# slcs-jsc/jurassic-gpu

Measured on AMD Instinct MI355X. Metric: rays/s (radiance spectra/s) for limb EGA forward model, higher is better.
Workload: dtype f64; 1 GPU; limb_1e6; rays_total=1000000, channels=4, emitters=5, tables=synthetic 33p x 10T x ~203u per (gas, channel), fp32

## Files before the change

include/jurassic_hip.h:

```cpp
#ifndef JURASSIC_HIP_H
#define JURASSIC_HIP_H

#include "jurassic_abi.h"

#ifdef __cplusplus
extern "C" {
#endif

void formod(ctl_t const *ctl, atm_t *atm, obs_t *obs);
void formod_GPU(ctl_t const *ctl, atm_t *atm, obs_t *obs);
void formod_pencil(ctl_t const *ctl, atm_t *atm, obs_t *obs, int const ir);
void formod_contrib(ctl_t const *ctl, atm_t *atm, obs_t *obs, obs_t *contrib);
void formod_fov(ctl_t const *ctl, obs_t *obs);

void intpol_atm(ctl_t *ctl, atm_t *atm_dest, atm_t *atm_src);

typedef struct { size_t size1, size2, tda; double *data; void *block; int owner; } jur_gsl_matrix_t;
void kernel(ctl_t const *ctl, atm_t *atm, obs_t *obs, jur_gsl_matrix_t *k);

enum {
  JUR_OK = 0,
  JUR_EINVAL = -1,
  JUR_EIO = -2,
  JUR_ENOMEM = -3,
// ... 59 lines not shown
int  jur_curtis_godson_host(jur_model_t *m, long nr, double const *const geom[7],
                            double *cgp, double *cgt, double *cgu, double *const tp[3], int *np_out);

int  jur_fov_read_shape(char const *filename, int *n, double *dz, double *w);
int  jur_fov_apply(int nd, long nr, double const *time, double const *vpz, double *rad, double *tau, long ld,
                   int n, double const *dz, double const *w);

int  jur_fov_apply_device(jur_model_t *m, long nr, double const *d_time, double const *d_vpz, double *d_rad,
                          double *d_tau, int n, double const *dz, double const *w, void *stream);

int  jur_intpol_atm(ctl_t const *ctl, atm_t *dest, atm_t const *src, int device);

int  jur_model_reserve(jur_model_t *m, long nr);

long jur_model_workspace_bytes(jur_model_t const *m);
int  jur_model_chunk_rays(jur_model_t const *m);
long jur_model_table_bytes(jur_model_t const *m);
int  jur_device_info(int device, char *pci_bus_id, int len, size_t *free_bytes, size_t *total_bytes);
int  jur_model_set_chunk_rays(jur_model_t *m, int rays);
int  jur_model_set_sort_rays(jur_model_t *m, int on);
int  jur_model_set_trace_multiple(jur_model_t *m, int mult);
int  jur_model_set_compact_workspace(jur_model_t *m, int on);
long jur_model_last_launches(jur_model_t const *m);
int  jur_model_set_workspace_budget(jur_model_t *m, long bytes);

int  jur_model_set_pencil(jur_model_t *m, long max_rays, int rays_per_group);
void jur_tune_trace(int lanes_per_ray);
void jur_tune_combine(int channels_per_group, int sync_segments, long min_lanes);

enum { JUR_ARITH_FAST = 0, JUR_ARITH_EXACT = 1 };
int  jur_model_set_arithmetic(jur_model_t *m, int mode);
int  jur_model_arithmetic(jur_model_t const *m);

int  jur_dropin_finalize(void);

int  jur_model_enable_timing(jur_model_t *m, int on);
int  jur_model_last_kernel_ms(jur_model_t *m, double out_ms[3], long out_launches[3]);
int  jur_model_last_pencil_ms(jur_model_t *m, double *out_ms, long *out_launches);
int  jur_model_last_contrib_ms(jur_model_t *m, double *out_ms, long *out_launches);

int jur_kat_ega_eps(jur_model_t *m, int ig, int id, long n, double const *tau, double const *t, double const *u,
                    double const *p, int mode, int chain, double *out);
int jur_kat_continua(jur_model_t *m, int id, long n, double const *p, double const *t, double const *q,
                     double const *u_co2, double const *u_h2o, double *out);
int jur_kat_update(jur_model_t *m, int id, long n, int what, double const *a, double const *b, double const *c,
                   double *rad, double *tau, double *src);
// ... 8 lines not shown
```

jurassic-gpu_amd/csrc/jur_internal.h:

```cpp
#ifndef JUR_INTERNAL_H
#define JUR_INTERNAL_H

#include <stdint.h>
#include "jurassic_hip.h"

#ifdef __cplusplus
extern "C" {
#endif

typedef struct { int a, b; } jur_int2;
typedef struct { float u, eps; } jur_ue_t;
typedef struct { float u0, e0, u1, e1; double du_de, de_du; } __attribute__((aligned(32))) jur_rec_t;
typedef struct { double p; int nt; int c0; } jur_lvl_t;
typedef struct { double t; int nu; int e0; } jur_crv_t;

typedef struct {
  double nu;
  double co2_cw296, co2_cw260, co2_cw230;
  double h2o_sc;
  double h2o_ratio;
  double h2o_lnr_hi, h2o_lnr_lo;
  double h2o_ctwfrn;
  double n2_b, n2_beta;
  double o2_b, o2_beta;
// ... 26 lines not shown
  int atm_sorted;
  double const *atm_time, *atm_z, *atm_lon, *atm_lat, *atm_p, *atm_t;
  double const *atm_q;
  double const *atm_k;
  double const *atm_pslope;
} jur_view_t;

typedef struct {
  int n;
  int stride;
  int stride_eps;
  long first;
  int const *order;
  double const *geom[7];
  double *tp[3];
  double *rad, *tau;
  int *np_out;
  int *np;
  double *tsurf;
  double *los;
  double *eps;
  int const *eps_off;
  int *status;
} jur_chunk_t;

int jurk_prepare_atm(jur_view_t const *v, double *d_pslope, void *stream);
int jurk_launch_trace(jur_view_t const *v, jur_chunk_t const *c, void *stream);
int jurk_launch_ega(jur_view_t const *v, jur_chunk_t const *c, void *stream);
int jurk_launch_combine(jur_view_t const *v, jur_chunk_t const *c, void *stream);
int jurk_launch_contrib(jur_view_t const *v, jur_chunk_t const *c, long nr, double *rad_c, double *tau_c, void *stream);
int jurk_tile_max(int n, int const *d_np, int *d_tile_np, void *stream);
int jurk_launch_kquot(long nq, long n, double const *d_rad, double const *d_h, double *d_kq, void *stream);
void jurk_tune_combine(int group, int sync, long min_lanes);
void jurk_tune_trace(int lanes);
int jurk_launch_cg(jur_view_t const *v, jur_chunk_t const *c, double *cgp, double *cgt, double *cgu, void *stream);
int jurk_fill_records(jur_ue_t const *ue, jur_rec_t *rec, long long n, void *stream);
long jurk_sort_tmp_bytes(long nr);
int jurk_sort_rays(jur_view_t const *v, int by_profile, long nr, double const *d_geom, long ld, int *d_order, void *tmp,
                   long tmp_bytes, void *stream);

long jurk_pencil_lds_bytes(jur_view_t const *v, int RB);
int jurk_launch_pencil(jur_view_t const *v, jur_chunk_t const *c, int RB, void *stream);

int jurk_launch_fov(long nr, int nd, double const *time, double const *vpz, double const *rad0, double const *tau0, double *rad,
                    double *tau, long ld, int n, double const *dz, double const *w, int *status, void *stream);

int jurk_launch_intpol(int ip, int ng, int nw, int ns, int nd_, int nx, double cx, double cz, double const *src, double const *x1,
                       int const *idx, int const *nz, double const *dst, double const *x0, double *out, void *stream);

int jurk_kat_ega(jur_view_t const *v, int g, int d, long n, double const *tau, double const *t, double const *u, double const *p,
                 int mode, int chain, double *out, void *stream);
int jurk_kat_continua(jur_view_t const *v, int d, long n, double const *p, double const *t, double const *q, double const *u_co2,
                      double const *u_h2o, double *out, void *stream);
int jurk_kat_update(jur_view_t const *v, int d, long n, int what, double const *a, double const *b, double const *c, double *rad,
// ... 63 lines not shown
```

jurassic-gpu_amd/csrc/jur_kernels.hip:

```cpp

#include <hip/hip_runtime.h>
#include <hipcub/hipcub.hpp>
#include <cstdlib>
#include <mutex>
#include "jur_internal.h"

#define NLOS JUR_NLOS
#define TBLNS JUR_TBLNS

namespace {

__device__ __forceinline__ double c01(double x) { return (x > 1.) ? 1. : ((x < 0.) ? 0. : x); }
__device__ __forceinline__ double c01_num(double x) { return __builtin_fmax(__builtin_fmin(x, 1.), 0.); }

__device__ __forceinline__ double lip(double x0, double y0, double x1, double y1, double x) {
  return y0 + (x - x0) * (y1 - y0) / (x1 - x0);
}

__device__ __forceinline__ double div_rcp(double a, double b, double r) {
  double const q = a * r;
  return __builtin_fma(__builtin_fma(-b, q, a), r, q);
}
__device__ __forceinline__ double lip_rcp(double x0, double y0, double x1, double y1, double x, double r) {
  return y0 + div_rcp((x - x0) * (y1 - y0), x1 - x0, r);
// ... 1007 lines not shown
  int const npair = v.nd * v.ng;
  BlockItem const bi = xcd_block_item((int)blockIdx.x, nrb, npair);
  int const rb = bi.rb, pr = bi.item;
  if (rb < 0) return;
  int const d = pr / v.ng, g = pr - d * v.ng;
  int const r = rb * blockDim.x + threadIdx.x;
  int const pair_idx = g * v.nd + d;
  jur_int2 const pd = v.pair[pair_idx];
  if (pd.a < 2) return;
  PairDesc<LDS> D{v.lvl, v.crv, v.ue + v.pair_e0[pair_idx], (unsigned)pd.b, 0u, 0u, 0u};
  if constexpr (RCPB) D.recb = v.rec + v.pair_e0[pair_idx];
  stage_pair<LDS, RCPB>(v, pd, D);
  if (r >= c.n) return;
  int const nfield = JUR_F_K + v.nw + v.ng;
  int const tile = __builtin_amdgcn_readfirstlane(r >> 6);
  unsigned const lane = (unsigned)(r & 63);
  size_t const R = (size_t)nfield * 64;
  double const *const los_tile = c.los + (size_t)tile * los_tile_doubles(nfield);
  double const *const los_p = los_tile + JUR_F_P * 64, *const los_t = los_tile + JUR_F_T * 64,
               *const los_u = los_tile + (size_t)(JUR_F_K + v.nw + g) * 64;
  size_t const Re = (size_t)npair * 64;
  double *const out = c.eps + eps_tile_point0(c, tile) * Re + (size_t)pr * 64;
  int const np = c.np[r];
  double tau_path = 1.0;
  unsigned br = 0, ia = 0, ib = 0;
  constexpr bool AHEAD = RCPB || !WARM;
  double p_next = 0., t_next = 0.;
  if (AHEAD && np > 0) { p_next = ldg<double>(los_p, lane); t_next = ldg<double>(los_t, lane); }

  for (int ip = 0; ip < np; ++ip) {
    size_t const o = (size_t)ip * R;
    double p, t;
    if constexpr (AHEAD) {
      p = p_next; t = t_next;
      if (ip + 1 < np) { p_next = ldg<double>(los_p + o + R, lane); t_next = ldg<double>(los_t + o + R, lane); }
    } else { p = ldg<double>(los_p + o, lane); t = ldg<double>(los_t + o, lane); }
    double const u = ldg<double>(los_u + o, lane);
    if constexpr (RCPB) tau_path = ega_eps_warm<LDS, true, true>(v, pd, D, tau_path, t, u, p, br, ia, ib);
    else if constexpr (WARM) tau_path *= ega_eps_warm<LDS, false>(v, pd, D, tau_path, t, u, p, br, ia, ib);
    else tau_path *= ega_eps_exact<LDS>(v, pd, D, tau_path, t, u, p);
    st_stream(out + (size_t)ip * Re, lane, tau_path);
  }
}

struct SegmentIn { double p, t, ds, k, u_co2, q_h2o, u_h2o, pcur; };
__device__ __forceinline__ SegmentIn load_segment(double const *__restrict__ row, double const *__restrict__ trow, unsigned lane,
                                                  int f_k, int f_co2, int f_h2o, int ng, unsigned has_table) {
  SegmentIn in;
  in.p = ldg<double>(row + JUR_F_P * 64, lane);
  in.t = ldg<double>(row + JUR_F_T * 64, lane);
  in.ds = ldg<double>(row + JUR_F_DS * 64, lane);
  in.k = ldg<double>(row + (size_t)f_k * 64, lane);
  in.u_co2 = ldg<double>(row + (size_t)f_co2 * 64, lane);
  in.q_h2o = ldg<double>(row + JUR_F_QH2O * 64, lane);
  in.u_h2o = ldg<double>(row + (size_t)f_h2o * 64, lane);
  double tg[8];
#pragma unroll
  for (int k = 0; k < 8; k++) tg[k] = (k < ng && ((has_table >> k) & 1u)) ? ld_stream(trow + (size_t)k * 64, lane) : 1.0;
  double pcur = 1.0;
#pragma unroll
  for (int k = 0; k < 8; k++) pcur *= tg[k];
  for (int g0 = 8; g0 < ng; g0 += 8) {
#pragma unroll
    for (int k = 0; k < 8; k++) tg[k] = (g0 + k < ng && g0 + k < 32 && ((has_table >> (g0 + k)) & 1u)) ? ld_stream(trow + (size_t)(g0 + k) * 64, lane) : 1.0;
// ... 13 lines not shown
  double *const sr = reinterpret_cast<double *>(jur_lds);
  Exp2Lds const e2t{sr + TBLNS};
  {
    double const *const gsr = v.sr + (size_t)d * TBLNS;
    for (int i = threadIdx.x; i < TBLNS; i += blockDim.x) sr[i] = gsr[i];
    if (threadIdx.x < 64) sr[TBLNS + threadIdx.x] = JUR_EXP2_64[threadIdx.x];
    __syncthreads();
  }
  if (r >= c.n) return;
  long const ray = c.order ? (long)c.order[r] : c.first + r;
  int const nfield = JUR_F_K + v.nw + ng;
  int const tile = __builtin_amdgcn_readfirstlane(r >> 6);
  unsigned const lane = (unsigned)(r & 63);
  size_t const R = (size_t)nfield * 64, Re = (size_t)nd * ng * 64;
  double const *const los = c.los + (size_t)tile * los_tile_doubles(nfield);
  double const *const epsb = c.eps + eps_tile_point0(c, tile) * Re + (size_t)d * ng * 64;
  jur_chan_t const ch = v.chan[d];
  int const f_k = JUR_F_K + ch.window, f_u = JUR_F_K + v.nw;
  bool const do_co2 = (v.fourbit & 8) && ch.co2_on, do_h2o = (v.fourbit & 4) && ch.h2o_on,
             do_n2 = (v.fourbit & 2) && ch.n2_on, do_o2 = (v.fourbit & 1) && ch.o2_on;
  size_t const oidx = (size_t)ray * nd + d;
  bool const masked = !isfinite(c.rad[oidx]);
  double rad = 0.0, tau = 1.0, pprev = 1.0;
  int const np = c.np[r];
  unsigned has_table = 0;
  for (int g = 0; g < ng && g < 32; g++) has_table |= (v.pair[g * nd + d].a >= 2 ? 1u : 0u) << g;
  int const f_co2 = do_co2 ? f_u + v.ig_co2 : JUR_F_P, f_h2o = do_h2o ? f_u + v.ig_h2o : JUR_F_P;
  for (int ip = 0; ip < np; ++ip) {
    SegmentIn const in = load_segment(los + (size_t)ip * R, epsb + (size_t)ip * Re, lane, f_k, f_co2, f_h2o, ng, has_table);
    double beta_ds = in.k * in.ds;
    if (do_co2) beta_ds += ctm_co2(ch, in.p, in.t, in.u_co2);
    double const rt = rcp_t(in.t);
    if (do_h2o) beta_ds += ctm_h2o(e2t, ch, in.p, in.t, rt, in.q_h2o, in.u_h2o);
    if (do_n2) beta_ds += ctm_n2(e2t, ch, in.p, in.t, rt) * in.ds;
    if (do_o2) beta_ds += ctm_o2(e2t, ch, in.p, in.t, rt) * in.ds;
    double const tau_gas = segment_tau_gas(in.pcur, pprev);
    pprev = in.pcur;
    new_obs_step(e2t, tau_gas, beta_ds, planck_src(sr, in.t), rad, tau);
  }
  ray_epilogue(sr, ch.nu, c.tsurf[r], v.write_bbt, rad, tau);
  if (masked) rad = __builtin_nan("");
  c.rad[oidx] = rad;
  c.tau[oidx] = tau;
}

#ifndef JUR_COMBINE_WAVES
#define JUR_COMBINE_WAVES 8
// ... 2 lines not shown
  int const nd = v.nd, ng = v.ng;
  int const ncg = (nd + CG - 1) / CG, SUB = (int)(blockDim.x >> 6) / CG;
  BlockItem const bi = xcd_block_item((int)blockIdx.x, nsb, ncg);
  int const sb = bi.rb, cg = bi.item;
  if (sb < 0) return;
  int const w = __builtin_amdgcn_readfirstlane((int)(threadIdx.x >> 6)), lane = (int)(threadIdx.x & 63);
  int const cw = w % CG, sub = w / CG;
  int const d = cg * CG + cw;
  bool const live_wave = d < nd;
  double *const sr = reinterpret_cast<double *>(jur_lds) + (size_t)cw * TBLNS;
  int *const npmax_sh = reinterpret_cast<int *>(reinterpret_cast<double *>(jur_lds) + (size_t)CG * TBLNS);
  Exp2Lds const e2t{reinterpret_cast<double *>(jur_lds) + (size_t)CG * TBLNS + 2};
  if (threadIdx.x == 0) *npmax_sh = 0;
  if (threadIdx.x < 64) reinterpret_cast<double *>(jur_lds)[(size_t)CG * TBLNS + 2 + threadIdx.x] = JUR_EXP2_64[threadIdx.x];
  for (int k = 0; k < CG; k++) {
    if (cg * CG + k >= nd) break;
    double const *const gsr = v.sr + (size_t)(cg * CG + k) * TBLNS;
    double *const dst = reinterpret_cast<double *>(jur_lds) + (size_t)k * TBLNS;
    for (int i = threadIdx.x; i < TBLNS; i += blockDim.x) dst[i] = gsr[i];
  }
  __syncthreads();
  int const r = (sb * SUB + sub) * 64 + lane;
  bool const live = live_wave && r < c.n;
  int const np = live ? c.np[r] : 0;
  atomicMax(npmax_sh, np);
  __syncthreads();
  int const npmax = *npmax_sh;
  long const ray = live ? (c.order ? (long)c.order[r] : c.first + r) : 0;
  int const nfield = JUR_F_K + v.nw + ng;
  int const tile = sb * SUB + sub;
  size_t const R = (size_t)nfield * 64, Re = (size_t)nd * ng * 64;
  double const *const los = c.los + (size_t)tile * los_tile_doubles(nfield);
  int const dd = live_wave ? d : 0;
  double const *const epsb = c.eps + eps_tile_point0(c, tile) * Re + (size_t)dd * ng * 64;
  jur_chan_t const ch = v.chan[dd];
  int const f_k = JUR_F_K + ch.window, f_u = JUR_F_K + v.nw;
  bool const do_co2 = (v.fourbit & 8) && ch.co2_on, do_h2o = (v.fourbit & 4) && ch.h2o_on,
             do_n2 = (v.fourbit & 2) && ch.n2_on, do_o2 = (v.fourbit & 1) && ch.o2_on;
  size_t const oidx = (size_t)ray * nd + dd;
  bool const masked = live && !isfinite(c.rad[oidx]);
  double rad = 0.0, tau = 1.0, pprev = 1.0;
  unsigned has_table = 0;
  for (int g = 0; g < ng && g < 32; g++) has_table |= (v.pair[g * nd + dd].a >= 2 ? 1u : 0u) << g;
  int const f_co2 = do_co2 ? f_u + v.ig_co2 : JUR_F_P, f_h2o = do_h2o ? f_u + v.ig_h2o : JUR_F_P;
  for (int ip = 0; ip < npmax; ++ip) {
    if (ip < np) {
      SegmentIn const in = load_segment(los + (size_t)ip * R, epsb + (size_t)ip * Re, (unsigned)lane, f_k, f_co2, f_h2o, ng, has_table);
// ... 390 lines not shown
  }
}

__global__ __launch_bounds__(256) void jur_records_kernel(long long n, jur_ue_t const *__restrict__ ue, jur_rec_t *__restrict__ rec) {
  for (long long i = (long long)blockIdx.x * blockDim.x + threadIdx.x; i < n; i += (long long)gridDim.x * blockDim.x) {
    double const du = (double)ue[i + 1].u - (double)ue[i].u, de = (double)ue[i + 1].eps - (double)ue[i].eps;
    rec[i] = jur_rec_t{ue[i].u, ue[i].eps, ue[i + 1].u, ue[i + 1].eps, du / de, de / du};
  }
}

__global__ __launch_bounds__(256) void jur_kquot_kernel(long nq, long n, long nrnd, double const *__restrict__ rad,
                                                        double const *__restrict__ h, double *__restrict__ kq) {
  long const t = (long)blockIdx.x * blockDim.x + threadIdx.x;
  if (t >= nq * n) return;
  long const q = t / n, e = t - q * n;
  kq[t] = (rad[(e + 1) * nrnd + q] - rad[q]) / h[e];
}

__global__ __launch_bounds__(256) void jur_tilemax_kernel(int n, int const *__restrict__ np, int *__restrict__ tile_np) {
  int const r = blockIdx.x * blockDim.x + threadIdx.x;
  int m = r < n ? np[r] : 0;
  for (int o = 32; o > 0; o >>= 1) m = max(m, __shfl_xor(m, o));
  if ((threadIdx.x & 63) == 0 && (r >> 6) < (n + 63) / 64) tile_np[r >> 6] = m;
}

__global__ __launch_bounds__(256) void jur_raykey_kernel(long nr, long ld, double const *__restrict__ geom,
                                                         double const *__restrict__ atm_time, int atm_np, int by_profile,
                                                         unsigned long long *__restrict__ key, int *__restrict__ id) {
  long const r = (long)blockIdx.x * blockDim.x + threadIdx.x;
  if (r >= nr) return;
  double xo[3], xv[3], e[3];
  geo2cart(geom[1 * ld + r], geom[2 * ld + r], geom[3 * ld + r], xo);
  geo2cart(geom[4 * ld + r], geom[5 * ld + r], geom[6 * ld + r], xv);
  for (int i = 0; i < 3; i++) e[i] = xv[i] - xo[i];
  double const n = norm3(e);
  double h = norm3(xo) - JUR_RE;
  if (n > 0) {
    double s = 0;
    for (int i = 0; i < 3; i++) s -= xo[i] * e[i] / n;
    if (s > 0) h = sqrt(fmax(xo[0] * xo[0] + xo[1] * xo[1] + xo[2] * xo[2] - s * s, 0.)) - JUR_RE;
  }
  unsigned const fb = __float_as_uint((float)h);
  unsigned const ord = fb ^ ((fb >> 31) ? 0xffffffffu : 0x80000000u);
  unsigned long long slice = 0;
  if (by_profile) {
    double const time = geom[r];
// ... 282 lines not shown
  if (c->n <= 0) return 0;
  int const block = 256;
  int const nrb = (c->n + block - 1) / block;
  long const nitem = (long)v->nd * (v->ng + 1);
  if (((long)(nrb >> 3) + 1) * 8 * nitem * block >= (1L << 32)) return (int)hipErrorInvalidValue;
  unsigned const grid = xcd_grid(nrb, (int)nitem);
  hipLaunchKernelGGL(jur_contrib_kernel, dim3(grid), dim3(block), sizeof(double) * (JUR_TBLNS + 64), (hipStream_t)stream, *v, *c,
                     nrb, nr, rad_c, tau_c);
  return (int)hipGetLastError();
}

extern "C" int jurk_launch_kquot(long nq, long n, double const *d_rad, double const *d_h, double *d_kq, void *stream) {
  if (nq <= 0 || n <= 0) return 0;
  hipLaunchKernelGGL(jur_kquot_kernel, dim3((unsigned)((nq * n + 255) / 256)), dim3(256), 0, (hipStream_t)stream, nq, n, nq, d_rad, d_h, d_kq);
  return (int)hipGetLastError();
}

extern "C" int jurk_tile_max(int n, int const *d_np, int *d_tile_np, void *stream) {
  if (n <= 0) return 0;
  hipLaunchKernelGGL(jur_tilemax_kernel, dim3((unsigned)((n + 255) / 256)), dim3(256), 0, (hipStream_t)stream, n, d_np, d_tile_np);
  return (int)hipGetLastError();
}

extern "C" int jurk_launch_cg(jur_view_t const *v, jur_chunk_t const *c, double *cgp, double *cgt, double *cgu,
                              void *stream) {
  if (c->n <= 0 || v->ng <= 0) return 0;
  int const block = 256;
  long const pencils = (long)c->n * v->ng;
  unsigned const grid = (unsigned)((pencils * 64 + block - 1) / block);
  hipLaunchKernelGGL(jur_cg_kernel, dim3(grid), dim3(block), 0, (hipStream_t)stream, *v, *c, cgp, cgt, cgu);
  return (int)hipGetLastError();
}

static size_t align_up(size_t x) { return (x + 255) & ~(size_t)255; }

extern "C" long jurk_sort_tmp_bytes(long nr) {
  size_t cub = 0;
  if (hipcub::DeviceRadixSort::SortPairs(nullptr, cub, (unsigned long long const *)nullptr, (unsigned long long *)nullptr,
                                         (int const *)nullptr, (int *)nullptr, (int)nr) != hipSuccess)
    cub = 64 * (size_t)nr + (1 << 20);
  return (long)(2 * align_up(8 * (size_t)nr) + align_up(4 * (size_t)nr) + align_up(cub) + 256);
}

extern "C" int jurk_sort_rays(jur_view_t const *v, int by_profile, long nr, double const *d_geom, long ld, int *d_order, void *tmp,
                              long tmp_bytes, void *stream) {
  hipStream_t s = (hipStream_t)stream;
// ... 125 lines not shown
```

jurassic-gpu_amd/csrc/jur_model.c:

```c
#define _GNU_SOURCE
#include <math.h>
#include <stdio.h>
#include <stdlib.h>
#include <string.h>
#include <strings.h>
#include <pthread.h>
#include <unistd.h>
#include <sched.h>
#include <hip/hip_runtime_api.h>
#include "jur_internal.h"

#define HIPCHK(call)                                                                       \
  do {                                                                                     \
    hipError_t e_ = (call);                                                                \
    if (e_ != hipSuccess) {                                                                \
      jur_set_error("HIP error %d (%s) at %s:%d", (int)e_, hipGetErrorString(e_), __FILE__, __LINE__); \
      return JUR_EHIP;                                                                     \
    }                                                                                      \
  } while (0)

struct jur_model {
  int device;
  int shared_tables;
  ctl_t *ctl;
  jur_view_t view;
  long table_bytes;
  void *d_chan, *d_sr, *d_pair, *d_pair_e0, *d_lvl, *d_crv, *d_ue, *d_rec;
  int arith;
  void *d_atm;
  int atm_cap;
  int atm_slices;
  double atm_zmin, atm_zmax;
  int chunk_rays;
  int nfield;
  double *d_los;
  double *d_eps;
  long ws_budget;
  long ws_rays;
  long ws_trace_rays;
  int trace_mult;
  long use_rays, use_trace_rays;
  int *d_np;
  double *d_tsurf;
  int compact_ws;
  int use_compact;
  int *d_tile_np, *d_eps_off;
  int *h_tile;
  long n_launch_ega;
  int *d_status;
  long los_bytes;
  int sort_rays;
  int *d_order;
  void *d_sort_tmp;
  long order_cap, sort_tmp_bytes;
  double *d_io;
  int *d_io_np;
  long io_cap;
  int *h_status;
  double *h_io;
  long h_io_cap;
  double *h_pkg;
  double *h_atm;
  long h_atm_n, h_atm_cap;
  double h_atm_hydz;
  hipStream_t stream;
  hipStream_t stream2;
  hipEvent_t ev_mask, ev_trace;
  int host_call;
  hipEvent_t ev_done;
// ... 122 lines not shown
    }
    v->rec = (jur_rec_t const *)m->d_rec;
  }
  v->sorted_tables = fl.sorted;
  v->strict_tables = fl.strict;
  v->max_pair_curves = fl.max_pair_curves;
  m->table_bytes = (long)((sizeof(jur_ue_t) + (m->d_rec ? sizeof(jur_rec_t) : 0)) * fl.nentry + 16 * fl.ncurve + 16 * fl.nlevel + 8 * npair);
  jur_flat_free(&fl);
  if (rc) { jur_model_destroy(m); return rc; }
  v->chan = (jur_chan_t const *)m->d_chan;
  v->sr = (double const *)m->d_sr;
  v->pair = (jur_int2 const *)m->d_pair;
  v->pair_e0 = (long long const *)m->d_pair_e0;
  v->lvl = (jur_lvl_t const *)m->d_lvl;
  v->crv = (jur_crv_t const *)m->d_crv;
  v->ue = (jur_ue_t const *)m->d_ue;
  if ((rc = jur_model_set_arithmetic(m, getenv("JUR_EGA_NO_RCP") ? JUR_ARITH_EXACT : JUR_ARITH_FAST))) { jur_model_destroy(m); return rc; }

  m->nfield = JUR_F_K + v->nw + v->ng;
  m->chunk_rays = 1 << 21;
  m->sort_rays = 1;
  m->ws_budget = 128L << 30;
  m->compact_ws = getenv("JUR_NO_COMPACT_WS") ? 0 : 1;
  m->trace_mult = 1;
  m->pencil_rays = 10000;
  m->pencil_rb = 0;
  if (getenv("JUR_PENCIL_RAYS")) m->pencil_rays = atol(getenv("JUR_PENCIL_RAYS"));
  if (getenv("JUR_PENCIL_RB")) m->pencil_rb = atoi(getenv("JUR_PENCIL_RB"));
  if (getenv("JUR_CHUNK_RAYS") && atoi(getenv("JUR_CHUNK_RAYS")) >= 64) m->chunk_rays = (atoi(getenv("JUR_CHUNK_RAYS")) + 63) / 64 * 64;
  if (getenv("JUR_TRACE_MULT") && atoi(getenv("JUR_TRACE_MULT")) >= 1) m->trace_mult = atoi(getenv("JUR_TRACE_MULT"));
  if (getenv("JUR_WS_GIB") && atoi(getenv("JUR_WS_GIB")) >= 1) m->ws_budget = (long)atoi(getenv("JUR_WS_GIB")) << 30;
  if ((rc = create_streams(m))) { jur_model_destroy(m); return rc; }
  if ((rc = upload((void **)&m->d_status, NULL, sizeof(int)))) { jur_model_destroy(m); return rc; }
  if (hipMemset(m->d_status, 0, sizeof(int)) != hipSuccess) { jur_set_error("cannot clear the status word"); jur_model_destroy(m); return JUR_EHIP; }
  *out = m;
  return JUR_OK;
}

int jur_model_set_arithmetic(jur_model_t *m, int mode) {
  if (mode != JUR_ARITH_FAST && mode != JUR_ARITH_EXACT) { jur_set_error("set_arithmetic: JUR_ARITH_FAST or JUR_ARITH_EXACT"); return JUR_EINVAL; }
  jur_view_t *v = &m->view;
  int const lds_ok = v->max_pair_curves > 0 && 24L * JUR_TBLNP + 24L * v->max_pair_curves <= 48 * 1024;
  m->arith = mode;
  v->fast_arith = (mode == JUR_ARITH_FAST) && v->strict_tables && v->rec && lds_ok;
  return JUR_OK;
}
// ... 201 lines not shown
    return JUR_OK;
  }
  if ((long)(nrow * n) > m->h_atm_cap) {
    free(m->h_atm);
    m->h_atm = (double *)malloc(sizeof(double) * nrow * n);
    m->h_atm_cap = m->h_atm ? (long)(nrow * n) : 0;
  }
  m->h_atm_n = 0;
  if (m->h_atm) { memcpy(m->h_atm, h, sizeof(double) * nrow * n); m->h_atm_n = n; m->h_atm_hydz = m->ctl->hydz; }
  hydrostatic_rows(m, h, (size_t)n, 0, n);
  int const rc = upload_atm_rows(m, h, n);
  if (rc) m->h_atm_n = 0;
  free(h);
  return rc;
}

static void free_workspace(jur_model_t *m) {
  if (m->d_los) (void)hipFree(m->d_los);
  if (m->d_eps) (void)hipFree(m->d_eps);
  if (m->d_np) (void)hipFree(m->d_np);
  if (m->d_tsurf) (void)hipFree(m->d_tsurf);
  if (m->d_tile_np) (void)hipFree(m->d_tile_np);
  if (m->d_eps_off) (void)hipFree(m->d_eps_off);
  if (m->h_tile) (void)hipHostFree(m->h_tile);
  m->d_los = NULL; m->d_eps = NULL; m->d_np = NULL; m->d_tsurf = NULL; m->d_tile_np = NULL; m->d_eps_off = NULL; m->h_tile = NULL;
  m->los_bytes = 0; m->ws_rays = 0; m->ws_trace_rays = 0;
}

static int ensure_workspace(jur_model_t *m, long nr) {
  long const per_ray_los = (long)sizeof(double) * m->nfield * JUR_NLOS;
  long const per_ray_eps = (long)sizeof(double) * m->view.nd * (m->view.ng > 0 ? m->view.ng : 1) * JUR_NLOS;
  long budget = m->ws_budget;
  int asked = 0;
  for (int attempt = 0;; attempt++) {
    long R = m->chunk_rays;
    long const fit = budget / (per_ray_los + per_ray_eps);
    if (R > fit) R = fit / 64 * 64;
    if (R < 64) R = 64;
    if (nr <= R) R = (nr + 63) / 64 * 64;
    else {
      long const nchunk = (nr + R - 1) / R;
      R = ((nr + nchunk - 1) / nchunk + 63) / 64 * 64;
    }
    long mult = m->trace_mult > 0 ? m->trace_mult : 1;
    while (mult > 1 && (per_ray_los * mult + per_ray_eps) * R > budget) mult--;
    long Rt = R * mult;
    if (nr < Rt) Rt = (nr + R - 1) / R * R;
    int compact = 0;
    if (nr > R && m->compact_ws) {
      long Rt_c = (nr + 63) / 64 * 64;
      if (per_ray_los * Rt_c > budget / 2) Rt_c = budget / 2 / per_ray_los / 64 * 64;
      long R_c = (budget - per_ray_los * Rt_c) / per_ray_eps / 64 * 64;
      if (R_c > m->chunk_rays) R_c = m->chunk_rays;
      if (R_c >= 64 && Rt_c >= R_c) { R = R_c; Rt = Rt_c; compact = 1; }
    }
    if (R <= m->ws_rays && Rt <= m->ws_trace_rays) {
      m->use_rays = R;
      m->use_trace_rays = Rt;
      m->use_compact = compact;
      return JUR_OK;
    }
    if (!asked) {
      size_t free_b = 0, total_b = 0;
      asked = 1;
      if (hipMemGetInfo(&free_b, &total_b) == hipSuccess) {
        long const avail = (long)free_b + m->los_bytes - (2L << 30);
        if (avail > (64L << 20) && avail < budget) { budget = avail; continue; }
      } else (void)hipGetLastError();
    }
    free_workspace(m);
    hipError_t e = hipMalloc((void **)&m->d_los, (size_t)per_ray_los * Rt);
    if (e == hipSuccess) e = hipMalloc((void **)&m->d_eps, (size_t)per_ray_eps * R);
    if (e == hipSuccess) e = hipMalloc((void **)&m->d_np, sizeof(int) * Rt);
    if (e == hipSuccess) e = hipMalloc((void **)&m->d_tsurf, sizeof(double) * Rt);
    if (e == hipSuccess) e = hipMalloc((void **)&m->d_tile_np, sizeof(int) * (Rt / 64 + 1));
    if (e == hipSuccess) e = hipMalloc((void **)&m->d_eps_off, sizeof(int) * (Rt / 64 + 1));
    if (e == hipSuccess) e = hipHostMalloc((void **)&m->h_tile, sizeof(int) * 2 * (Rt / 64 + 1), hipHostMallocDefault);
    if (e == hipSuccess) {
      m->los_bytes = per_ray_los * Rt + per_ray_eps * R;
      m->ws_rays = R;
      m->ws_trace_rays = Rt;
      m->use_rays = R;
      m->use_trace_rays = Rt;
      m->use_compact = compact;
      return JUR_OK;
    }
    (void)hipGetLastError();
    free_workspace(m);
    if (R <= 64 || attempt >= 24) {
      jur_set_error("cannot allocate the workspace (%ld B per ray, even for %ld rays): %s", per_ray_los + per_ray_eps, R,
                    hipGetErrorString(e));
      return JUR_EHIP;
    }
    budget = (per_ray_los + per_ray_eps) * R / 2;
// ... 4 lines not shown
long jur_model_table_bytes(jur_model_t const *m) { return m->table_bytes; }

int jur_device_info(int device, char *pci_bus_id, int len, size_t *free_bytes, size_t *total_bytes) {
  int ndev = 0;
  if (hipGetDeviceCount(&ndev) != hipSuccess || device < 0 || device >= ndev) { jur_set_error("device %d not available", device); return JUR_ENODEV; }
  HIPCHK(hipSetDevice(device));
  if (pci_bus_id && len > 0) HIPCHK(hipDeviceGetPCIBusId(pci_bus_id, len, device));
  size_t f = 0, t = 0;
  HIPCHK(hipMemGetInfo(&f, &t));
  if (free_bytes) *free_bytes = f;
  if (total_bytes) *total_bytes = t;
  return JUR_OK;
}
int jur_model_device(jur_model_t const *m) { return m->device; }
int jur_model_nd(jur_model_t const *m) { return m->view.nd; }
void *jur_model_stream(jur_model_t const *m) { return (void *)m->stream; }
int *jur_model_status_word(jur_model_t const *m) { return m->d_status; }
void jur_model_cost_params(jur_model_t const *m, double *rayds, double *raydz, double *zmin, double *zmax) {
  *rayds = m->view.rayds; *raydz = m->view.raydz; *zmin = m->atm_zmin; *zmax = m->atm_zmax;
}
int jur_model_chunk_rays(jur_model_t const *m) { return m->chunk_rays; }
long jur_model_last_launches(jur_model_t const *m) { return m->n_launch_ega; }
int jur_model_set_compact_workspace(jur_model_t *m, int on) { m->compact_ws = on ? 1 : 0; return JUR_OK; }

int jur_model_set_sort_rays(jur_model_t *m, int on) { m->sort_rays = on ? 1 : 0; return JUR_OK; }

int jur_model_set_workspace_budget(jur_model_t *m, long bytes) {
  if (bytes < (64L << 20)) { jur_set_error("workspace budget below 64 MiB"); return JUR_EINVAL; }
  m->ws_budget = bytes;
  return JUR_OK;
}

int jur_model_set_trace_multiple(jur_model_t *m, int mult) {
  if (mult < 1 || mult > 64) { jur_set_error("trace multiple must be in 1..64"); return JUR_EINVAL; }
  m->trace_mult = mult;
  return JUR_OK;
}

int jur_model_set_chunk_rays(jur_model_t *m, int rays) {
  if (rays < 64 || rays > (1 << 22)) { jur_set_error("chunk_rays must be in 64..4194304"); return JUR_EINVAL; }
  m->chunk_rays = (rays + 63) / 64 * 64;
  return JUR_OK;
}

int jur_model_set_pencil(jur_model_t *m, long max_rays, int rays_per_group) {
  if (max_rays < 0 || rays_per_group < 0 || rays_per_group > 64) { jur_set_error("set_pencil: max_rays >= 0, rays_per_group in 0..64"); return JUR_EINVAL; }
// ... 156 lines not shown
  }
  rc = ensure_workspace(m, nr);
  if (rc) return rc;
  long const R = m->use_rays;
  int const *order = NULL;
  if (m->sort_rays && nr > 64) {
    rc = ensure_sort_buffers(m, nr);
    if (rc) return rc;
    int const by_profile = m->atm_slices > 1 && nr >= 1024L * m->atm_slices;
    int const e = jurk_sort_rays(&m->view, by_profile, nr, d_geom, ldg, m->d_order, m->d_sort_tmp, m->sort_tmp_bytes, s);
    if (e) { jur_set_error("ray sort failed: %s", hipGetErrorString((hipError_t)e)); return JUR_EHIP; }
    order = m->d_order;
  }
  long const Rt = m->use_trace_rays;
  m->n_launch_ega = 0;
#define TIMED(kind, launch, what)                                                              \
  do {                                                                                         \
    int const ti_ = (m->timing && m->ntimed < JUR_MAX_TIMED) ? m->ntimed++ : -1;               \
    if (ti_ >= 0) { m->evkind[ti_] = (kind); HIPCHK(hipEventRecord(m->evpool[2 * ti_], s)); } \
    int const e_ = (launch);                                                                   \
    if (e_) { jur_set_error(what " kernel launch failed: %s", hipGetErrorString((hipError_t)e_)); return JUR_EHIP; } \
    if (ti_ >= 0) HIPCHK(hipEventRecord(m->evpool[2 * ti_ + 1], s));                          \
  } while (0)
  for (long t0 = 0; t0 < nr; t0 += Rt) {
    jur_chunk_t c;
    long const nt = (nr - t0 < Rt) ? nr - t0 : Rt;
    c.stride = (int)Rt;
    c.stride_eps = (int)R;
    for (int k = 0; k < 7; k++) c.geom[k] = d_geom + (size_t)k * ldg;
    for (int k = 0; k < 3; k++) c.tp[k] = d_tp + (size_t)k * ldtp;
    c.rad = d_rad;
    c.tau = d_tau;
    c.np_out = d_np;
    c.eps = m->d_eps;
    c.status = d_status ? d_status : m->d_status;
    c.n = (int)nt;
    c.first = t0;
    c.order = order ? order + t0 : NULL;
    c.np = m->d_np;
    c.tsurf = m->d_tsurf;
    c.los = m->d_los;
    TIMED(0, jurk_launch_trace(&m->view, &c, s), "trace");
    if (m->host_call) {
      if (t0 == 0) HIPCHK(hipStreamWaitEvent(s, m->ev_mask, 0));
      if (t0 + Rt >= nr) HIPCHK(hipEventRecord(m->ev_trace, s));
    }
    c.eps_off = NULL;
    int compact = m->use_compact && nt > R;
    if (compact) {
      hipStreamCaptureStatus st = hipStreamCaptureStatusNone;
      if (hipStreamIsCapturing(s, &st) != hipSuccess) { (void)hipGetLastError(); st = hipStreamCaptureStatusNone; }
      if (st != hipStreamCaptureStatusNone) compact = 0;
    }
    if (compact) {
      long const ntile = (nt + 63) / 64, cap = R / 64 * JUR_NLOS;
      int *const h_np = m->h_tile, *const h_off = m->h_tile + (m->ws_trace_rays / 64 + 1);
      int const ek = jurk_tile_max((int)nt, m->d_np, m->d_tile_np, s);
      if (ek) { jur_set_error("tile kernel launch failed: %s", hipGetErrorString((hipError_t)ek)); return JUR_EHIP; }
// ... 3 lines not shown
      for (long t = 0; t < ntile; t++) total += h_np[t];
      long const nchunk = (total + cap - 1) / cap > 0 ? (total + cap - 1) / cap : 1;
      long const target = (total + nchunk - 1) / nchunk;
      for (long t = 0; t < ntile;) {
        long acc = 0, e = t;
        while (e < ntile && (e == t || (acc + h_np[e] <= cap && acc < target))) acc += h_np[e++];
        if (e < ntile && e - t >= 64) e = t + (e - t) / 32 * 32;
        acc = 0;
        for (long q = t; q < e; q++) { h_off[q] = (int)acc; acc += h_np[q]; h_np[q] = (q == t); }
        t = e;
      }
      HIPCHK(hipMemcpyAsync(m->d_eps_off, h_off, sizeof(int) * ntile, hipMemcpyHostToDevice, s));
      for (long t0c = 0; t0c < ntile;) {
        long t1c = t0c + 1;
        while (t1c < ntile && !h_np[t1c]) t1c++;
        long const s0 = t0c * 64, s1 = (t1c * 64 < nt) ? t1c * 64 : nt;
        c.n = (int)(s1 - s0);
        c.first = t0 + s0;
        c.order = order ? order + t0 + s0 : NULL;
        c.np = m->d_np + s0;
        c.tsurf = m->d_tsurf + s0;
        c.los = m->d_los + (size_t)s0 * JUR_NLOS * m->nfield;
        c.eps_off = m->d_eps_off + t0c;
        TIMED(1, jurk_launch_ega(&m->view, &c, s), "ega");
        if (co) TIMED(4, jurk_launch_contrib(&m->view, &c, nr, co->rad, co->tau, s), "contribution");
        TIMED(2, jurk_launch_combine(&m->view, &c, s), "combine");
        m->n_launch_ega++;
        t0c = t1c;
      }
      continue;
    }
    for (long s0 = 0; s0 < nt; s0 += R) {
      c.n = (int)((nt - s0 < R) ? nt - s0 : R);
      c.first = t0 + s0;
      c.order = order ? order + t0 + s0 : NULL;
      c.np = m->d_np + s0;
      c.tsurf = m->d_tsurf + s0;
      c.los = m->d_los + (size_t)s0 * JUR_NLOS * m->nfield;
      TIMED(1, jurk_launch_ega(&m->view, &c, s), "ega");
      if (co) TIMED(4, jurk_launch_contrib(&m->view, &c, nr, co->rad, co->tau, s), "contribution");
      TIMED(2, jurk_launch_combine(&m->view, &c, s), "combine");
      m->n_launch_ega++;
    }
  }
#undef TIMED
  return record_done(m, s);
}

void *jur_host_alloc(size_t bytes) {
  void *p = NULL;
  if (hipHostMalloc(&p, bytes ? bytes : 8, hipHostMallocDefault) != hipSuccess) {
    (void)hipGetLastError();
    jur_set_error("hipHostMalloc of %zu bytes failed", bytes);
    return NULL;
  }
  return p;
}
void jur_host_free(void *p) { if (p) (void)hipHostFree(p); }

static int is_pinned(void const *p) {
  hipPointerAttribute_t a;
  if (!p) return 0;
  if (hipPointerGetAttributes(&a, p) != hipSuccess) { (void)hipGetLastError(); return 0; }
  return a.type == hipMemoryTypeHost;
}

typedef struct { char *dst; char const *src; size_t n; } cpjob_t;
static void *cp_worker(void *a) { cpjob_t const *j = (cpjob_t const *)a; memcpy(j->dst, j->src, j->n); return NULL; }
// ... 882 lines not shown
```

jurassic-gpu_amd/jurassic_hip/lib.py:

```python
import ctypes as C
import os
import numpy as np
from . import abi

PKG = os.path.dirname(os.path.dirname(os.path.abspath(__file__)))
SO = os.environ.get("JURASSIC_HIP_SO",
                    os.path.join(PKG, "libjurassic_hip%s.so" % os.environ.get("JUR_SUFFIX", "")))
_lib = None
dp = C.POINTER(C.c_double)


class JurassicError(RuntimeError):
    pass


def lib():
    global _lib
    if _lib is None:
        if not os.path.exists(SO):
            raise JurassicError(f"{SO} not built: run `make -C jurassic-gpu_amd/csrc` "
                                "or __graft_entry__.build(); no CPU fallback exists")
        L = C.CDLL(SO)
        L.jur_last_error.restype = C.c_char_p
        L.jur_fov_read_shape.argtypes = [C.c_char_p, C.POINTER(C.c_int), dp, dp]
# ... 22 lines not shown
        L.jur_curtis_godson_host.argtypes = [C.c_void_p, C.c_long, C.POINTER(dp), dp, dp, dp, C.POINTER(dp), C.POINTER(C.c_int)]
        L.jur_fov_apply_device.argtypes = [C.c_void_p, C.c_long] + [C.c_void_p] * 4 + [C.c_int, dp, dp, C.c_void_p]
        L.jur_intpol_atm.argtypes = [C.c_void_p, C.c_void_p, C.c_void_p, C.c_int]
        L.intpol_atm.argtypes = [C.c_void_p] * 3
        L.intpol_atm.restype = None
        L.jur_host_alloc.restype = C.c_void_p
        L.jur_host_alloc.argtypes = [C.c_size_t]
        L.jur_host_free.argtypes = [C.c_void_p]
        L.jur_formod_device.argtypes = [C.c_void_p, C.c_long] + [C.c_void_p] * 7
        L.jur_formod_contrib_host.argtypes = [C.c_void_p, C.c_long, C.POINTER(dp), dp, dp, C.POINTER(dp), C.POINTER(C.c_int), dp, dp]
        L.jur_formod_contrib_device.argtypes = [C.c_void_p, C.c_long] + [C.c_void_p] * 9
        L.formod_contrib.argtypes = [C.c_void_p] * 4
        L.formod_contrib.restype = None
        L.jur_model_reserve.argtypes = [C.c_void_p, C.c_long]
        L.jur_model_workspace_bytes.restype = C.c_long
        L.jur_model_workspace_bytes.argtypes = [C.c_void_p]
        L.jur_model_table_bytes.restype = C.c_long
        L.jur_model_table_bytes.argtypes = [C.c_void_p]
        L.jur_device_info.argtypes = [C.c_int, C.c_char_p, C.c_int, C.POINTER(C.c_size_t), C.POINTER(C.c_size_t)]
        L.jur_model_chunk_rays.argtypes = [C.c_void_p]
        L.jur_model_last_launches.restype = C.c_long
        L.jur_model_last_launches.argtypes = [C.c_void_p]
        L.jur_model_set_compact_workspace.argtypes = [C.c_void_p, C.c_int]
        L.jur_model_set_chunk_rays.argtypes = [C.c_void_p, C.c_int]
        L.jur_model_set_sort_rays.argtypes = [C.c_void_p, C.c_int]
        L.jur_model_set_trace_multiple.argtypes = [C.c_void_p, C.c_int]
        L.jur_model_set_workspace_budget.argtypes = [C.c_void_p, C.c_long]
        L.jur_model_enable_timing.argtypes = [C.c_void_p, C.c_int]
        L.jur_model_last_kernel_ms.argtypes = [C.c_void_p, dp, C.POINTER(C.c_long)]
        L.jur_model_last_pencil_ms.argtypes = [C.c_void_p, dp, C.POINTER(C.c_long)]
        L.jur_model_last_contrib_ms.argtypes = [C.c_void_p, dp, C.POINTER(C.c_long)]
        L.jur_model_set_pencil.argtypes = [C.c_void_p, C.c_long, C.c_int]
        L.jur_model_set_arithmetic.argtypes = [C.c_void_p, C.c_int]
        L.jur_model_arithmetic.argtypes = [C.c_void_p]
        L.jur_multi_balance.argtypes = [C.c_void_p, C.c_long, C.POINTER(dp), C.c_int, C.POINTER(C.c_long)]
        L.jur_estimate_los_points.argtypes = [C.c_double] * 4 + [C.c_long, C.POINTER(dp), dp]
        L.jur_balance_rays.argtypes = [C.c_double] * 4 + [C.c_long, C.POINTER(dp), C.c_int, C.POINTER(C.c_long)]
        L.jur_models_set_atm.argtypes = [C.POINTER(C.c_void_p), C.c_int, C.c_void_p]
        L.jur_formod_host_multi.argtypes = [C.POINTER(C.c_void_p), C.c_int, C.c_long, C.POINTER(dp), dp, dp, C.POINTER(dp), C.POINTER(C.c_int)]
        L.jur_formod_device_multi.argtypes = [C.POINTER(C.c_void_p), C.c_int, C.c_long, C.POINTER(C.c_long)] + [C.c_void_p] * 7
        L.jur_tune_combine.argtypes = [C.c_int, C.c_int, C.c_long]
        L.jur_tune_combine.restype = None
        L.jur_tune_trace.argtypes = [C.c_int]
        L.jur_tune_trace.restype = None
        L.jur_state_size.restype = C.c_size_t
        L.jur_state_size.argtypes = [C.c_void_p, C.c_void_p]
# ... 271 lines not shown
    def kernel_ms(self):
        ms = (C.c_double * 3)()
        n = (C.c_long * 3)()
        _chk(lib().jur_model_last_kernel_ms(self.h, ms, n))
        pm, pn = C.c_double(0), C.c_long(0)
        _chk(lib().jur_model_last_pencil_ms(self.h, C.byref(pm), C.byref(pn)))
        return dict(trace_ms=ms[0], ega_ms=ms[1], combine_ms=ms[2], trace_launches=n[0], ega_launches=n[1],
                    combine_launches=n[2], pencil_ms=pm.value, pencil_launches=pn.value)

    def contrib_ms(self):
        ms, n = C.c_double(0), C.c_long(0)
        _chk(lib().jur_model_last_contrib_ms(self.h, C.byref(ms), C.byref(n)))
        return dict(contrib_ms=ms.value, contrib_launches=n.value)

    def workspace_bytes(self):
        return lib().jur_model_workspace_bytes(self.h)

    def last_launches(self):
        return lib().jur_model_last_launches(self.h)

    def set_compact_workspace(self, on):
        _chk(lib().jur_model_set_compact_workspace(self.h, int(on)))

    def table_bytes(self):
        return lib().jur_model_table_bytes(self.h)


ARITH_FAST, ARITH_EXACT = 0, 1
ENLOS = -5


class GslMatrix(C.Structure):
    _fields_ = [("size1", C.c_size_t), ("size2", C.c_size_t), ("tda", C.c_size_t), ("data", dp), ("block", C.c_void_p),
                ("owner", C.c_int)]


def kernel(ctl, atm, obs, m, n, tda=None):
    tda = tda or n
    store = np.full((m, tda), -7.0)
    mat = GslMatrix(m, n, tda, _p(store), None, 0)
    lib().kernel(C.byref(ctl), C.byref(atm), C.byref(obs), C.byref(mat))
    assert np.all(store[:, n:] == -7.0)
    return store[:, :n].copy()


def device_info(device):
# ... 106 lines not shown
```

Measured before the change: 19.07 million rays/s.

## Stop EGA path integration once transmittance becomes opaque, shared across gases

Adds an opaque-exit mode, on by default. A per-(channel, ray) cutoff index is reset by a new arming kernel before each EGA launch. In the EGA kernel, a gas lane that sees path transmittance drop below 1e-9 records its point index with an atomic min and stops. The other gas lanes of the same ray poll that index every fourth point and shorten their loop to it, and the combine kernels cap each ray's point count there too. The aim is to skip table lookups and eps stores for path points behind an opaque segment. The cost is an extra launch, atomics and polling loads, plus slightly different results because contributions below the threshold are dropped.

```diff
diff --git a/include/jurassic_hip.h b/include/jurassic_hip.h
--- a/include/jurassic_hip.h
+++ b/include/jurassic_hip.h
@@ -105,6 +105,8 @@
 int  jur_model_set_trace_multiple(jur_model_t *m, int mult);
 int  jur_model_set_compact_workspace(jur_model_t *m, int on);
 long jur_model_last_launches(jur_model_t const *m);
+int  jur_model_set_opaque_exit(jur_model_t *m, int on);
+int  jur_model_last_live(jur_model_t *m, int *out, long cap, long *nslot);
 int  jur_model_set_workspace_budget(jur_model_t *m, long bytes);
 
 int  jur_model_set_pencil(jur_model_t *m, long max_rays, int rays_per_group);
diff --git a/jurassic-gpu_amd/csrc/jur_internal.h b/jurassic-gpu_amd/csrc/jur_internal.h
--- a/jurassic-gpu_amd/csrc/jur_internal.h
+++ b/jurassic-gpu_amd/csrc/jur_internal.h
@@ -72,6 +72,8 @@
   double *eps;
   int const *eps_off;
   int *status;
+  int *last;
+  int stride_last;
 } jur_chunk_t;
 
 int jurk_prepare_atm(jur_view_t const *v, double *d_pslope, void *stream);
@@ -80,6 +82,7 @@
 int jurk_launch_combine(jur_view_t const *v, jur_chunk_t const *c, void *stream);
 int jurk_launch_contrib(jur_view_t const *v, jur_chunk_t const *c, long nr, double *rad_c, double *tau_c, void *stream);
 int jurk_tile_max(int n, int const *d_np, int *d_tile_np, void *stream);
+int jurk_arm_last(int *d_last, long n, void *stream);
 int jurk_launch_kquot(long nq, long n, double const *d_rad, double const *d_h, double *d_kq, void *stream);
 void jurk_tune_combine(int group, int sync, long min_lanes);
 void jurk_tune_trace(int lanes);
diff --git a/jurassic-gpu_amd/csrc/jur_kernels.hip b/jurassic-gpu_amd/csrc/jur_kernels.hip
--- a/jurassic-gpu_amd/csrc/jur_kernels.hip
+++ b/jurassic-gpu_amd/csrc/jur_kernels.hip
@@ -1053,24 +1053,34 @@
   size_t const Re = (size_t)npair * 64;
   double *const out = c.eps + eps_tile_point0(c, tile) * Re + (size_t)pr * 64;
   int const np = c.np[r];
+  int *const lastp = c.last ? c.last + (size_t)d * c.stride_last + r : nullptr;
+  bool const poll = lastp && v.ng > 1;
+  int lim = np - 1;
   double tau_path = 1.0;
   unsigned br = 0, ia = 0, ib = 0;
   constexpr bool AHEAD = RCPB || !WARM;
   double p_next = 0., t_next = 0.;
   if (AHEAD && np > 0) { p_next = ldg<double>(los_p, lane); t_next = ldg<double>(los_t, lane); }
 
-  for (int ip = 0; ip < np; ++ip) {
+  for (int ip = 0; ip <= lim; ++ip) {
     size_t const o = (size_t)ip * R;
     double p, t;
     if constexpr (AHEAD) {
       p = p_next; t = t_next;
-      if (ip + 1 < np) { p_next = ldg<double>(los_p + o + R, lane); t_next = ldg<double>(los_t + o + R, lane); }
+      if (ip < lim) { p_next = ldg<double>(los_p + o + R, lane); t_next = ldg<double>(los_t + o + R, lane); }
     } else { p = ldg<double>(los_p + o, lane); t = ldg<double>(los_t + o, lane); }
     double const u = ldg<double>(los_u + o, lane);
+    int seen = 0x7f7f7f7f;
+    if (poll && (ip & 3) == 3) seen = __hip_atomic_load(lastp, __ATOMIC_RELAXED, __HIP_MEMORY_SCOPE_AGENT);
     if constexpr (RCPB) tau_path = ega_eps_warm<LDS, true, true>(v, pd, D, tau_path, t, u, p, br, ia, ib);
     else if constexpr (WARM) tau_path *= ega_eps_warm<LDS, false>(v, pd, D, tau_path, t, u, p, br, ia, ib);
     else tau_path *= ega_eps_exact<LDS>(v, pd, D, tau_path, t, u, p);
     st_stream(out + (size_t)ip * Re, lane, tau_path);
+    if (lastp && tau_path < 1e-9) {
+      __hip_atomic_fetch_min(lastp, ip, __ATOMIC_RELAXED, __HIP_MEMORY_SCOPE_AGENT);
+      break;
+    }
+    lim = min(lim, seen);
   }
 }
 
@@ -1130,7 +1140,7 @@
   size_t const oidx = (size_t)ray * nd + d;
   bool const masked = !isfinite(c.rad[oidx]);
   double rad = 0.0, tau = 1.0, pprev = 1.0;
-  int const np = c.np[r];
+  int const np = c.last ? min(c.np[r], c.last[(size_t)d * c.stride_last + r] + 1) : c.np[r];
   unsigned has_table = 0;
   for (int g = 0; g < ng && g < 32; g++) has_table |= (v.pair[g * nd + d].a >= 2 ? 1u : 0u) << g;
   int const f_co2 = do_co2 ? f_u + v.ig_co2 : JUR_F_P, f_h2o = do_h2o ? f_u + v.ig_h2o : JUR_F_P;
@@ -1179,7 +1189,8 @@
   __syncthreads();
   int const r = (sb * SUB + sub) * 64 + lane;
   bool const live = live_wave && r < c.n;
-  int const np = live ? c.np[r] : 0;
+  int np = live ? c.np[r] : 0;
+  if (live && c.last) np = min(np, c.last[(size_t)d * c.stride_last + r] + 1);
   atomicMax(npmax_sh, np);
   __syncthreads();
   int const npmax = *npmax_sh;
@@ -1616,6 +1627,11 @@
   int m = r < n ? np[r] : 0;
   for (int o = 32; o > 0; o >>= 1) m = max(m, __shfl_xor(m, o));
   if ((threadIdx.x & 63) == 0 && (r >> 6) < (n + 63) / 64) tile_np[r >> 6] = m;
+}
+
+__global__ __launch_bounds__(256) void jur_arm_last_kernel(long n, int *__restrict__ last) {
+  long const i = (long)blockIdx.x * blockDim.x + threadIdx.x;
+  if (i < n) last[i] = 0x7f7f7f7f;
 }
 
 __global__ __launch_bounds__(256) void jur_raykey_kernel(long nr, long ld, double const *__restrict__ geom,
@@ -1944,6 +1960,12 @@
   return (int)hipGetLastError();
 }
 
+extern "C" int jurk_arm_last(int *d_last, long n, void *stream) {
+  if (n <= 0) return 0;
+  hipLaunchKernelGGL(jur_arm_last_kernel, dim3((unsigned)((n + 255) / 256)), dim3(256), 0, (hipStream_t)stream, n, d_last);
+  return (int)hipGetLastError();
+}
+
 extern "C" int jurk_launch_cg(jur_view_t const *v, jur_chunk_t const *c, double *cgp, double *cgt, double *cgu,
                               void *stream) {
   if (c->n <= 0 || v->ng <= 0) return 0;
diff --git a/jurassic-gpu_amd/csrc/jur_model.c b/jurassic-gpu_amd/csrc/jur_model.c
--- a/jurassic-gpu_amd/csrc/jur_model.c
+++ b/jurassic-gpu_amd/csrc/jur_model.c
@@ -45,6 +45,9 @@
   int compact_ws;
   int use_compact;
   int *d_tile_np, *d_eps_off;
+  int opaque_exit;
+  int *d_last;
+  long last_n;
   int *h_tile;
   long n_launch_ega;
   int *d_status;
@@ -213,6 +216,7 @@
   m->sort_rays = 1;
   m->ws_budget = 128L << 30;
   m->compact_ws = getenv("JUR_NO_COMPACT_WS") ? 0 : 1;
+  m->opaque_exit = getenv("JUR_NO_OPAQUE_EXIT") ? 0 : 1;
   m->trace_mult = 1;
   m->pencil_rays = 10000;
   m->pencil_rb = 0;
@@ -460,13 +464,16 @@
   if (m->d_tsurf) (void)hipFree(m->d_tsurf);
   if (m->d_tile_np) (void)hipFree(m->d_tile_np);
   if (m->d_eps_off) (void)hipFree(m->d_eps_off);
+  if (m->d_last) (void)hipFree(m->d_last);
   if (m->h_tile) (void)hipHostFree(m->h_tile);
   m->d_los = NULL; m->d_eps = NULL; m->d_np = NULL; m->d_tsurf = NULL; m->d_tile_np = NULL; m->d_eps_off = NULL; m->h_tile = NULL;
+  m->d_last = NULL; m->last_n = 0;
   m->los_bytes = 0; m->ws_rays = 0; m->ws_trace_rays = 0;
 }
 
 static int ensure_workspace(jur_model_t *m, long nr) {
-  long const per_ray_los = (long)sizeof(double) * m->nfield * JUR_NLOS;
+  long const per_ray_last = (long)sizeof(int) * m->view.nd;
+  long const per_ray_los = (long)sizeof(double) * m->nfield * JUR_NLOS + per_ray_last;
   long const per_ray_eps = (long)sizeof(double) * m->view.nd * (m->view.ng > 0 ? m->view.ng : 1) * JUR_NLOS;
   long budget = m->ws_budget;
   int asked = 0;
@@ -507,7 +514,8 @@
       } else (void)hipGetLastError();
     }
     free_workspace(m);
-    hipError_t e = hipMalloc((void **)&m->d_los, (size_t)per_ray_los * Rt);
+    hipError_t e = hipMalloc((void **)&m->d_los, (size_t)(per_ray_los - per_ray_last) * Rt);
+    if (e == hipSuccess) e = hipMalloc((void **)&m->d_last, (size_t)per_ray_last * Rt);
     if (e == hipSuccess) e = hipMalloc((void **)&m->d_eps, (size_t)per_ray_eps * R);
     if (e == hipSuccess) e = hipMalloc((void **)&m->d_np, sizeof(int) * Rt);
     if (e == hipSuccess) e = hipMalloc((void **)&m->d_tsurf, sizeof(double) * Rt);
@@ -558,6 +566,19 @@
 int jur_model_chunk_rays(jur_model_t const *m) { return m->chunk_rays; }
 long jur_model_last_launches(jur_model_t const *m) { return m->n_launch_ega; }
 int jur_model_set_compact_workspace(jur_model_t *m, int on) { m->compact_ws = on ? 1 : 0; return JUR_OK; }
+
+int jur_model_set_opaque_exit(jur_model_t *m, int on) { m->opaque_exit = on ? 1 : 0; return JUR_OK; }
+
+int jur_model_last_live(jur_model_t *m, int *out, long cap, long *nslot) {
+  if (!m || !out || !nslot) { jur_set_error("last_live: bad arguments"); return JUR_EINVAL; }
+  *nslot = m->last_n;
+  if (m->last_n == 0) return JUR_OK;
+  if (cap < m->last_n * m->view.nd) { jur_set_error("last_live: room for %ld words, %ld needed", cap, m->last_n * m->view.nd); return JUR_EINVAL; }
+  HIPCHK(hipSetDevice(m->device));
+  HIPCHK(hipDeviceSynchronize());
+  HIPCHK(hipMemcpy(out, m->d_last, sizeof(int) * (size_t)(m->last_n * m->view.nd), hipMemcpyDeviceToHost));
+  return JUR_OK;
+}
 
 int jur_model_set_sort_rays(jur_model_t *m, int on) { m->sort_rays = on ? 1 : 0; return JUR_OK; }
 
@@ -760,6 +781,18 @@
     if (e_) { jur_set_error(what " kernel launch failed: %s", hipGetErrorString((hipError_t)e_)); return JUR_EHIP; } \
     if (ti_ >= 0) HIPCHK(hipEventRecord(m->evpool[2 * ti_ + 1], s));                          \
   } while (0)
+  int const use_last = m->opaque_exit && !co && m->view.ng > 0;
+  if (!use_last) m->last_n = 0;
+#define ARM_LAST()                                                                                           \
+  do {                                                                                                       \
+    if (use_last) {                                                                                          \
+      c.last = m->d_last;                                                                                    \
+      c.stride_last = (c.n + 63) / 64 * 64;                                                                  \
+      m->last_n = c.stride_last;                                                                             \
+      int const ea_ = jurk_arm_last(m->d_last, (long)c.stride_last * m->view.nd, s);                         \
+      if (ea_) { jur_set_error("arming kernel launch failed: %s", hipGetErrorString((hipError_t)ea_)); return JUR_EHIP; } \
+    }                                                                                                        \
+  } while (0)
   for (long t0 = 0; t0 < nr; t0 += Rt) {
     jur_chunk_t c;
     long const nt = (nr - t0 < Rt) ? nr - t0 : Rt;
@@ -772,6 +805,8 @@
     c.np_out = d_np;
     c.eps = m->d_eps;
     c.status = d_status ? d_status : m->d_status;
+    c.last = NULL;
+    c.stride_last = 0;
     c.n = (int)nt;
     c.first = t0;
     c.order = order ? order + t0 : NULL;
@@ -821,6 +856,7 @@
         c.tsurf = m->d_tsurf + s0;
         c.los = m->d_los + (size_t)s0 * JUR_NLOS * m->nfield;
         c.eps_off = m->d_eps_off + t0c;
+        ARM_LAST();
         TIMED(1, jurk_launch_ega(&m->view, &c, s), "ega");
         if (co) TIMED(4, jurk_launch_contrib(&m->view, &c, nr, co->rad, co->tau, s), "contribution");
         TIMED(2, jurk_launch_combine(&m->view, &c, s), "combine");
@@ -836,6 +872,7 @@
       c.np = m->d_np + s0;
       c.tsurf = m->d_tsurf + s0;
       c.los = m->d_los + (size_t)s0 * JUR_NLOS * m->nfield;
+      ARM_LAST();
       TIMED(1, jurk_launch_ega(&m->view, &c, s), "ega");
       if (co) TIMED(4, jurk_launch_contrib(&m->view, &c, nr, co->rad, co->tau, s), "contribution");
       TIMED(2, jurk_launch_combine(&m->view, &c, s), "combine");
@@ -843,6 +880,7 @@
     }
   }
 #undef TIMED
+#undef ARM_LAST
   return record_done(m, s);
 }
 
diff --git a/jurassic-gpu_amd/jurassic_hip/lib.py b/jurassic-gpu_amd/jurassic_hip/lib.py
--- a/jurassic-gpu_amd/jurassic_hip/lib.py
+++ b/jurassic-gpu_amd/jurassic_hip/lib.py
@@ -68,6 +68,8 @@
         L.jur_model_last_launches.restype = C.c_long
         L.jur_model_last_launches.argtypes = [C.c_void_p]
         L.jur_model_set_compact_workspace.argtypes = [C.c_void_p, C.c_int]
+        L.jur_model_set_opaque_exit.argtypes = [C.c_void_p, C.c_int]
+        L.jur_model_last_live.argtypes = [C.c_void_p, C.POINTER(C.c_int), C.c_long, C.POINTER(C.c_long)]
         L.jur_model_set_chunk_rays.argtypes = [C.c_void_p, C.c_int]
         L.jur_model_set_sort_rays.argtypes = [C.c_void_p, C.c_int]
         L.jur_model_set_trace_multiple.argtypes = [C.c_void_p, C.c_int]
@@ -385,6 +387,17 @@
     def set_compact_workspace(self, on):
         _chk(lib().jur_model_set_compact_workspace(self.h, int(on)))
 
+    def set_opaque_exit(self, on):
+        _chk(lib().jur_model_set_opaque_exit(self.h, int(on)))
+
+    def last_live(self, max_slots):
+        nd = self.nd
+        max_slots = (int(max_slots) + 63) // 64 * 64
+        buf = np.empty(nd * max_slots, dtype=np.int32)
+        n = C.c_long(0)
+        _chk(lib().jur_model_last_live(self.h, buf.ctypes.data_as(C.POINTER(C.c_int)), buf.size, C.byref(n)))
+        return buf[:nd * n.value].reshape(nd, n.value).copy() if n.value else None
+
     def table_bytes(self):
         return lib().jur_model_table_bytes(self.h)
 
```

Measured after the change: 19.34 million rays/s (median of 6 runs). 1.4% higher.
